# 530300865/Cooperative-ORB-SLAM

Measured on AMD Instinct MI355X. Metric: frames/sec ORB extract+match, 640x480 mono, 1000 feat/frame, higher is better.
Workload: dtype u8; 1 GPU; C2: synthetic 640x480 uint8, nfeatures 1000, scale 1.2, 8 levels, FAST 20/7; extract + BF SearchForTriangulation vs previous frame + per-step keyframe BoW + slot all-gather & cross-agent SearchForTriangulation and SearchByBoW(KF,KF); config=c2, stereo=False, graphs_per_gpu=3, graph_stagger=every8, scene=shared, exchange_stream=graph 0's, parallelism=agent-per-gpu x1

## Files before the change

cooperative-orb-slam_amd/csrc/launch.h:

```cpp
#pragma once
#include <hip/hip_runtime.h>
#include <stdint.h>

#include "../../include/orbslam_amd.h"
#include "orb_device.h"
#include "orb_frame.h"
#include "orb_match.h"
#include "orb_slot.h"

namespace orbamd {

hipError_t launch_resize(const uint8_t* src, long long src_fstride, int src_pitch, int sw, int sh, uint8_t* dst,
                         long long dst_fstride, int dst_pitch, int dw, int dh, const int* coef, int xmax,
                         int simd_end, int nframes, hipStream_t st);
hipError_t launch_pyramid_frames(const uint8_t* frames, long long fstride, int pitch0, uint8_t* pyr,
                                 const ExtractParams& ep, const LevelDesc* levels, const int* ptab, int max_rows,
                                 int max_groups, int nframes, hipStream_t st,
                                 const int2* bands = nullptr, int nbands = 0);
hipError_t launch_resize_tiled(const uint8_t* src, long long src_fstride, int src_pitch, int sw, int sh, uint8_t* dst,
                               long long dst_fstride, int dst_pitch, int dw, int dh, const int* coef, int xmax,
                               int simd_end, int nframes, hipStream_t st);
int resize_tile_fits(const int* xofs, const int* yofs, int sw, int sh, int dw, int dh);
hipError_t launch_fast_cells2(const uint8_t* frames, long long fstride, int pitch0, const uint8_t* pyr,
                              const ExtractParams& ep, const LevelDesc* levels, const CellDesc* cells,
                              uint32_t* cellkey, int* cellcnt, int RP, int RH, int max_pass, int cell_lo,
                              int cell_hi, int nframes, hipStream_t st);
hipError_t octree_setup(int lds_bytes);
hipError_t launch_sincos_selftest(const float* in, float* so, float* co, int n, hipStream_t st);
hipError_t launch_octree(const ExtractParams& ep, const LevelDesc* levels, const CellDesc* cells,
                         const uint32_t* cellkey, const int* cellcnt, uint32_t* lvkey, int* lvcnt,
                         uint8_t* gscratch, long long gscratch_frame_bytes, int NC, int KL, int lds_bytes,
                         int* err, int nframes, hipStream_t st, int level0 = 0, int nlevels = -1,
                         const HostCopy* copy = nullptr);
hipError_t launch_fast_blur(const uint8_t* frames, long long fstride, int pitch0, const uint8_t* pyr,
                            const ExtractParams& ep, const LevelDesc* levels, const CellDesc* cells, uint32_t* cellkey,
                            int* cellcnt, int RP, int RH, int max_pass, uint8_t* blur, const ExtractParams& eb,
                            int njobs, int nframes, hipStream_t st);
hipError_t launch_blur_strips(const uint8_t* frames, long long fstride, int pitch0, const uint8_t* pyr, uint8_t* blur,
                              const ExtractParams& ep, const LevelDesc* levels, int job0, int job1, const int* lvcnt,
                              int nframes, hipStream_t st, int rows = kBlurRows);
hipError_t launch_describe(const uint8_t* frames, long long fstride, int pitch0, const uint8_t* pyr,
                           const uint8_t* blur, const ExtractParams& ep, const LevelDesc* levels,
                           const uint32_t* lvkey, const int* lvcnt, orbx_kp* out_kps, uint8_t* out_desc,
                           int* out_counts, int kp_stride, const int* ptab, int nframes, hipStream_t st);
bool describe_blur_ok(const uint8_t* frames, long long fstride, int pitch0);
hipError_t launch_describe_blur(const uint8_t* frames, long long fstride, int pitch0, const uint8_t* pyr,
                                const ExtractParams& ep, const LevelDesc* levels, const uint32_t* lvkey,
                                const int* lvcnt, orbx_kp* out_kps, uint8_t* out_desc, int* out_counts, int kp_stride,
                                const int* ptab, int nframes, hipStream_t st);

hipError_t launch_tri_bf(int npairs, const int32_t* q1, const int32_t* q2, const orbx_kp* kps, const uint8_t* desc,
                         const int32_t* counts, int kp_stride, const MatchGeom& g, int32_t* match12,
                         int32_t* nmatches, hipStream_t st, const float* uright = nullptr, int only_stereo = 0);
hipError_t launch_tri_nodes_pairs(int npairs, int max_nodes, const int32_t* q1, const int32_t* q2, const orbx_kp* kps,
                                  const uint8_t* desc, int kp_stride, const uint32_t* fv_node, const int32_t* fv_off,
                                  const int32_t* fv_feat, const int32_t* nfv, const MatchGeom& g, int32_t* match12,
                                  int32_t* nmatches, hipStream_t st);
hipError_t launch_rot_filter_pairs(int npairs, const int32_t* q1, const int32_t* q2, const orbx_kp* kps,
                                   const int32_t* counts, int kp_stride, int32_t* match12, int32_t* nmatches,
                                   hipStream_t st, int swap = 0);
hipError_t launch_bow_pairs(int npairs, int max_nodes, const int32_t* qf, const int32_t* cf, const uint8_t* desc,
                            int kp_stride, const uint8_t* mp_flags, const uint32_t* fv_node, const int32_t* fv_off,
                            const int32_t* fv_feat, const int32_t* nfv, float nnratio, int mode, int32_t* out,
                            hipStream_t st);
hipError_t launch_count_pairs(int npairs, const int32_t* out, int kp_stride, int32_t* nmatches, hipStream_t st);
hipError_t launch_tri_nodes(const DevView& v1, const DevView& v2, const NodeTask* tasks, int ntasks,
                            const MatchGeom& g, int only_stereo, const CallTail& tail, hipStream_t st);
hipError_t launch_bow(const DevView& vq, const DevView& vc, const NodeTask* tasks, int ntasks, int max_nc,
                      float nnratio, int mode, const CallTail& tail, hipStream_t st);
hipError_t launch_bow_small(const BowSmall& a, hipStream_t st);
int proj_topk();
hipError_t launch_tri_small(const TriSmall& a, hipStream_t st);
hipError_t launch_rot_filter(int n, int32_t* m, const float* angA, const float* angB, int swap, int32_t* nout,
                             hipStream_t st);

hipError_t launch_undistort(const orbx_camera& cam, int nframes, const orbx_kp* kps, const int32_t* counts,
                            int kp_stride, orbx_kp* kps_un, float* kun, hipStream_t st);
hipError_t launch_undistort_deliver(const orbx_camera& cam, const orbx_kp* kps, const int32_t* count, int kp_stride,
                                    orbx_kp* raw_out, orbx_kp* un_out, int32_t* count_out, hipStream_t st);

hipError_t launch_unproject(float cx, float cy, float invfx, float invfy, int nframes, const orbx_kp* kps_un,
                            const float* depth, const int32_t* counts, int kp_stride, const float* Tcw, float* pos,
                            uint8_t* mp_flags, int valid_flags, hipStream_t st);
struct TrackArgs {
    const int32_t *cur, *last;
    int nframes;
// ... 75 lines not shown
```

cooperative-orb-slam_amd/csrc/match_kernels.hip:

```cpp
#include <hip/hip_runtime.h>
#include <stdint.h>
#include <limits.h>

#include "../../include/orbslam_amd.h"
#include "orb_match.h"
#include "orb_match_dev.h"
#include "orb_wave.h"

namespace orbamd {

__device__ __forceinline__ bool epi_ok_f(float a, float b, float c, float x2, float y2, float thf) {
    const float num = __fadd_rn(__fadd_rn(__fmul_rn(a, x2), __fmul_rn(b, y2)), c);
    const float den = __fadd_rn(__fmul_rn(a, a), __fmul_rn(b, b));
    if (den == 0.f) return false;
    const float dsqr = __fdiv_rn(__fmul_rn(num, num), den);
    return dsqr < thf;
}

__device__ __forceinline__ void epi_line(const MatchGeom& g, float x1, float y1, float* a, float* b, float* c) {
    epi_line(g.F, x1, y1, a, b, c);
}
__device__ __forceinline__ bool near_epipole(const MatchGeom& g, float x2, float y2, int oct2) {
    return near_epipole(g.ex, g.ey, x2, y2, g.th100[oct2]);
}

struct PairSrc {
    const orbx_kp* kps1; const uint8_t* desc1; int n1;
    const orbx_kp* kps2; const uint8_t* desc2; int n2;
    const float* ur1; const float* ur2;
};

typedef int v4i __attribute__((ext_vector_type(4)));

typedef int v8i __attribute__((ext_vector_type(8)));
typedef float v16f __attribute__((ext_vector_type(16)));
__device__ __forceinline__ uint32_t fp4_pm1_byte(uint32_t nb) {
    const uint32_t lo = nb & 15u, hi = (nb >> 4) & 15u;
    return ((hi * 0x10204080u) & 0x80808080u) | (((lo * 0x01020408u) & 0x08080808u) | 0x22222222u);
}
// ... 98 lines not shown
            auto key = [&](int p) {
                const float dp = __int_as_float(p & ~31);
                return ((uint32_t)(int)(256.f - dp) >> 1 << 16) + kb - (uint32_t)(p & 31);
            };
            int pmax = pk(0);
#pragma unroll
            for (int rg = 1; rg < 16; rg++) pmax = max(pmax, pk(rg));
            uint32_t km = key(pmax);
            while (km < best && (km >> 16) <= 50u) {
                const int jl = (int)(65535u - (km & 0xFFFFu)) - cb;
                const float4 c2 = s_rec[bf][jl];
                if ((!STEREO || st1 || c2.w == 0.0f) && epi_ok_f(la, lb, lc, c2.x, c2.y, c2.z)) {
                    best = km;
                    break;
                }
                const int cur = pmax;
                int nx = INT_MIN;
#pragma unroll
                for (int rg = 0; rg < 16; rg++) nx = pk(rg) < cur ? max(nx, pk(rg)) : nx;
                pmax = nx;
                km = nx == INT_MIN ? 0xFFFFFFFFu : key(nx);
            }
        }
        __syncthreads();
    }
    best = min(best, (uint32_t)__shfl_xor((int)best, 32, 64));
    if (qon && h == 0) {
        const int idx2 = qact && (best >> 16) <= 50u ? (int)(65535u - (best & 0xFFFFu)) : -1;
        out[qi] = idx2;
        if (idx2 >= 0) atomicAdd(nmatch, 1);
    }
}

#ifndef ORBX_MF_WPE
#define ORBX_MF_WPE 6
#endif
#define ORBX_MF_ATTR __attribute__((amdgpu_waves_per_eu(ORBX_MF_WPE)))
template <bool STEREO>
__global__ __launch_bounds__(kMfThreads) ORBX_MF_ATTR void k_tri_mfma(const int32_t* __restrict__ q1, const int32_t* __restrict__ q2,
                                                  const orbx_kp* __restrict__ kps, const uint8_t* __restrict__ desc,
                                                  const int32_t* __restrict__ counts, const float* __restrict__ uright,
                                                  int kp_stride, MatchGeom g, int only_stereo,
                                                  int32_t* __restrict__ match12, int32_t* __restrict__ nmatches) {
    const int p = blockIdx.y;
    const int f1 = q1[p], f2 = q2[p];
    PairSrc s;
    s.kps1 = kps + (long long)f1 * kp_stride; s.desc1 = desc + (long long)f1 * kp_stride * 32; s.n1 = counts[f1];
    s.kps2 = kps + (long long)f2 * kp_stride; s.desc2 = desc + (long long)f2 * kp_stride * 32; s.n2 = counts[f2];
    s.ur1 = STEREO ? uright + (long long)f1 * kp_stride : nullptr;
    s.ur2 = STEREO ? uright + (long long)f2 * kp_stride : nullptr;
    tri_mfma_body_fp4<STEREO>(s, g, match12 + (long long)p * kp_stride, nmatches + p, only_stereo);
}

__device__ __forceinline__ int rot_bin(const float* angA, const float* angB, int i, int j, int swap) {
    return swap ? rot_bin(angA[j], angB[i]) : rot_bin(angA[i], angB[j]);
}

__device__ __forceinline__ void call_emit(const CallTail& t, int i, int j) {
    const int bin = t.check_ori ? rot_bin(t.angA, t.angB, i, j, t.swap) : 0;
    if (t.check_ori) atomicAdd(t.state + 2 + bin, 1);
    const int k = atomicAdd(t.state + 1, 1);
    ((int4*)t.list)[k] = make_int4(i, j, bin, 0);
}

__device__ void call_tail(const CallTail& t) {
    __shared__ int s_last, s_cnt, s_nl;
    __shared__ int hist[30], keep[3];
    __syncthreads();
    __threadfence();
    if (threadIdx.x == 0) s_last = atomicAdd(t.state, 1) == (int)(gridDim.x - 1);
    __syncthreads();
    if (!s_last) return;
    __threadfence();
    if (threadIdx.x < 30) hist[threadIdx.x] = t.check_ori ? t.state[2 + threadIdx.x] : 0;
    if (threadIdx.x == 0) {
        s_cnt = 0;
        s_nl = t.state[1];
    }
    __syncthreads();
    if (threadIdx.x == 0) {
        if (t.check_ori) three_maxima(hist, keep);
        else keep[0] = keep[1] = keep[2] = -2;
    }
    __syncthreads();
// ... 390 lines not shown

__global__ __launch_bounds__(256) void k_rot_filter(int n, int32_t* __restrict__ m, const float* __restrict__ angA,
                                                    const float* __restrict__ angB, int swap, int32_t* __restrict__ nout) {
    __shared__ int hist[30];
    __shared__ int keep[3];
    const int local = rot_filter_rows(n, m, [&](int i, int j) { return rot_bin(angA, angB, i, j, swap); }, hist, keep);
    if (nout) atomicAdd(nout, local);
}

__global__ __launch_bounds__(256) void k_rot_filter_pairs(const int32_t* __restrict__ q1, const int32_t* __restrict__ q2,
                                                          const orbx_kp* __restrict__ kps, const int32_t* __restrict__ counts,
                                                          int kp_stride, int32_t* __restrict__ match12,
                                                          int32_t* __restrict__ nmatches, int swap) {
    __shared__ int hist[30];
    __shared__ int keep[3];
    const int p = blockIdx.x;
    const orbx_kp* k1 = kps + (long long)q1[p] * kp_stride;
    const orbx_kp* k2 = kps + (long long)q2[p] * kp_stride;
    if (threadIdx.x == 0) nmatches[p] = 0;
    const int local = rot_filter_rows(counts[q1[p]], match12 + (long long)p * kp_stride, [&](int i, int j) {
        return swap ? rot_bin(k2[j].angle, k1[i].angle) : rot_bin(k1[i].angle, k2[j].angle);
    }, hist, keep);
    atomicAdd(&nmatches[p], local);
}

}

#include "launch.h"

namespace orbamd {

hipError_t launch_tri_bf(int npairs, const int32_t* q1, const int32_t* q2, const orbx_kp* kps, const uint8_t* desc,
                         const int32_t* counts, int kp_stride, const MatchGeom& g, int32_t* match12,
                         int32_t* nmatches, hipStream_t st, const float* uright, int only_stereo) {
    if (npairs == 0) return hipSuccess;
    dim3 grid((kp_stride + 32 * kMfWaves - 1) / (32 * kMfWaves), npairs);
    if (uright)
        hipLaunchKernelGGL(k_tri_mfma<true>, grid, dim3(kMfThreads), 0, st, q1, q2, kps, desc, counts, uright, kp_stride,
                           g, only_stereo, match12, nmatches);
    else
        hipLaunchKernelGGL(k_tri_mfma<false>, grid, dim3(kMfThreads), 0, st, q1, q2, kps, desc, counts, uright,
                           kp_stride, g, 0, match12, nmatches);
    return hipGetLastError();
}

hipError_t launch_tri_nodes_pairs(int npairs, int max_nodes, const int32_t* q1, const int32_t* q2, const orbx_kp* kps,
                                  const uint8_t* desc, int kp_stride, const uint32_t* fv_node, const int32_t* fv_off,
                                  const int32_t* fv_feat, const int32_t* nfv, const MatchGeom& g, int32_t* match12,
                                  int32_t* nmatches, hipStream_t st) {
    if (npairs == 0 || max_nodes <= 0) return hipSuccess;
    hipLaunchKernelGGL(k_tri_nodes_pairs, dim3(max_nodes, npairs), dim3(64), 0, st, q1, q2, kps, desc, kp_stride,
                       fv_node, fv_off, fv_feat, nfv, g, match12, nmatches);
    return hipGetLastError();
}

hipError_t launch_rot_filter_pairs(int npairs, const int32_t* q1, const int32_t* q2, const orbx_kp* kps,
                                   const int32_t* counts, int kp_stride, int32_t* match12, int32_t* nmatches,
                                   hipStream_t st, int swap) {
    hipLaunchKernelGGL(k_rot_filter_pairs, dim3(npairs), dim3(256), 0, st, q1, q2, kps, counts, kp_stride, match12,
                       nmatches, swap);
    return hipGetLastError();
}

hipError_t launch_bow_pairs(int npairs, int max_nodes, const int32_t* qf, const int32_t* cf, const uint8_t* desc,
                            int kp_stride, const uint8_t* mp_flags, const uint32_t* fv_node, const int32_t* fv_off,
                            const int32_t* fv_feat, const int32_t* nfv, float nnratio, int mode, int32_t* out,
                            hipStream_t st) {
    if (npairs == 0 || max_nodes <= 0) return hipSuccess;
    hipLaunchKernelGGL(k_bow_pairs, dim3(max_nodes, npairs), dim3(64), (size_t)kp_stride, st, qf, cf, desc, kp_stride,
                       mp_flags, fv_node, fv_off, fv_feat, nfv, nnratio, mode, out);
    return hipGetLastError();
}

hipError_t launch_count_pairs(int npairs, const int32_t* out, int kp_stride, int32_t* nmatches, hipStream_t st) {
    if (npairs == 0) return hipSuccess;
// ... 42 lines not shown
```

cooperative-orb-slam_amd/csrc/matcher.cpp:

```cpp
#include "matcher_host.h"

using namespace orbamd;

namespace {

int wait_call(hipStream_t st, const int32_t* word) {
    return wait_until(st, [word] { return __atomic_load_n(word, __ATOMIC_ACQUIRE) >= 0; });
}

void make_geom(MatchGeom& g, const float F12[9], float ex, float ey, int nlevels, const float* scale,
               const float* sigma2) {
    for (int i = 0; i < 9; i++) g.F[i] = F12[i];
    g.ex = ex;
    g.ey = ey;
    for (int o = 0; o < 16; o++) {
        g.th100[o] = o < nlevels ? 100 * scale[o] : 0.f;
        g.th384[o] = o < nlevels ? 3.84 * (double)sigma2[o] : 0.0;
        float t = (float)g.th384[o];
        if ((double)t < g.th384[o]) t = std::nextafter(t, INFINITY);
        g.th384f[o] = t;
    }
}

void common_nodes(const orbm_kf_view* a, const orbm_kf_view* b, std::vector<std::pair<int, int>>& out) {
// ... 80 lines not shown
        if (p.octave != none) memcpy(hbase + p.octave, v->octave, 4 * n);
        if (p.uright != none) memcpy(hbase + p.uright, v->uright, 4 * n);
        if (v->has_mp) memcpy(hbase + p.has_mp, v->has_mp, n);
        if (v->mp_bad) memcpy(hbase + p.mp_bad, v->mp_bad, n);
    }
    if (p.nfeat) memcpy(hbase + p.feat, v->node_feat, 4 * (size_t)p.nfeat);
    return d;
}

}

extern "C" {

int orbm_create(int device, orbm_ctx** out) {
    if (!out) return ORBX_EARG;
    *out = nullptr;
    if (device < 0 || device >= orbx_device_count()) return ORBX_EDEVICE;
    HIPR(hipSetDevice(device));
    orbm_ctx* c = new orbm_ctx();
    c->device = device;
    if (c->err.ensure(256) || hipMemset(c->err.p, 0, 256) != hipSuccess) {
        orbm_destroy(c);
        return ORBX_EDEVICE;
    }
    *out = c;
    return 0;
}

void orbm_destroy(orbm_ctx* c) {
    if (!c) return;
    (void)hipSetDevice(c->device);
    if (c->stream) (void)hipStreamSynchronize(c->stream);
    c->scratch.release();
    c->err.release();
    if (c->pinned) (void)hipHostFree(c->pinned);
    if (c->stream) (void)hipStreamDestroy(c->stream);
    delete c;
}

int orbm_descriptor_distance(const uint8_t* a, const uint8_t* b) {
    if (!a || !b) return ORBX_EARG;
    int d = 0;
    for (int i = 0; i < 8; i++) {
        uint32_t x, y;
        memcpy(&x, a + 4 * i, 4);
        memcpy(&y, b + 4 * i, 4);
        d += __builtin_popcount(x ^ y);
    }
    return d;
}

void orbm_epipole(const float R2w[9], const float t2w[3], const float Cw[3], float fx, float fy, float cx, float cy,
                  float* ex, float* ey) {
    float C2[3];
    for (int i = 0; i < 3; i++) {
        const float* a = R2w + 3 * i;
        const float t0 = a[0] * Cw[0] + a[1] * Cw[1] + a[2] * Cw[2];
        C2[i] = (float)((double)t0 * 1.0 + (double)t2w[i] * 1.0);
    }
    const float invz = 1.0f / C2[2];
    *ex = fx * C2[0] * invz + cx;
    *ey = fy * C2[1] * invz + cy;
}

}

static int node_feats(const orbm_kf_view* v) { return v->n_nodes ? v->node_off[v->n_nodes] : 0; }

struct SmallSide {
    const uint4* d = nullptr;
// ... 281 lines not shown
    HIPR(launch_bow(dq, dc, (const NodeTask*)(base + o_tasks), (int)tasks.size(), max_nc, nnratio, mode, tail,
                    ctx->s()));
    if (const int rc = wait_call(ctx->s(), res)) return rc;
    memcpy(out, res + 1, 4 * (size_t)nout);
    if (nmatches) *nmatches = res[0];
    return 0;
}

int orbm_search_by_bow_kf_f(orbm_ctx* ctx, const orbm_kf_view* kf, const orbm_kf_view* f, float nnratio,
                            int check_ori, int32_t* match_f, int* nmatches) {
    if (!ctx || !view_ok(kf) || !view_ok(f) || !match_f) return ORBX_EARG;
    return bow_common(ctx, kf, f, nnratio, check_ori, 0, match_f, f->n, nmatches);
}

int orbm_search_by_bow_kf_kf(orbm_ctx* ctx, const orbm_kf_view* kf1, const orbm_kf_view* kf2, float nnratio,
                             int check_ori, int32_t* match12, int* nmatches) {
    if (!ctx || !view_ok(kf1) || !view_ok(kf2) || !match12) return ORBX_EARG;
    return bow_common(ctx, kf1, kf2, nnratio, check_ori, 1, match12, kf1->n, nmatches);
}

int orbm_triangulation_bf_batch_device(orbm_ctx* ctx, int npairs, const int32_t* d_q1, const int32_t* d_q2,
                                       const orbx_kp* d_kps, const uint8_t* d_desc, const int32_t* d_counts,
                                       int kp_stride, const float F12[9], float ex, float ey, int nlevels,
                                       const float* scale_factors, const float* level_sigma2, int check_ori,
                                       int32_t* d_match12, int32_t* d_nmatches, void* stream) {
    if (!ctx || npairs < 0 || !F12 || nlevels < 1 || nlevels > 16 || !scale_factors || !level_sigma2 ||
        kp_stride < 1 || kp_stride > 64 * 1024)
        return ORBX_EARG;
    if (npairs == 0) return 0;
    HIPR(hipSetDevice(ctx->device));
    MatchGeom g;
    make_geom(g, F12, ex, ey, nlevels, scale_factors, level_sigma2);
    hipStream_t st = (hipStream_t)stream;
    HIPR(hipMemsetAsync(d_nmatches, 0, sizeof(int32_t) * npairs, st));
    HIPR(launch_tri_bf(npairs, d_q1, d_q2, d_kps, d_desc, d_counts, kp_stride, g, d_match12, d_nmatches, st));
    if (check_ori)
        HIPR(launch_rot_filter_pairs(npairs, d_q1, d_q2, d_kps, d_counts, kp_stride, d_match12, d_nmatches, st));
    return 0;
}

int orbm_triangulation_bf_stereo_batch_device(orbm_ctx* ctx, int npairs, const int32_t* d_q1, const int32_t* d_q2,
                                              const orbx_kp* d_kps, const uint8_t* d_desc, const int32_t* d_counts,
                                              const float* d_uright, int kp_stride, const float F12[9], float ex,
                                              float ey, int nlevels, const float* scale_factors,
                                              const float* level_sigma2, int only_stereo, int check_ori,
                                              int32_t* d_match12, int32_t* d_nmatches, void* stream) {
    if (!ctx || npairs < 0 || !F12 || nlevels < 1 || nlevels > 16 || !scale_factors || !level_sigma2 ||
        kp_stride < 1 || kp_stride > 64 * 1024 || (npairs > 0 && !d_uright))
        return ORBX_EARG;
    if (npairs == 0) return 0;
    HIPR(hipSetDevice(ctx->device));
    MatchGeom g;
    make_geom(g, F12, ex, ey, nlevels, scale_factors, level_sigma2);
    hipStream_t st = (hipStream_t)stream;
    HIPR(hipMemsetAsync(d_nmatches, 0, sizeof(int32_t) * npairs, st));
    HIPR(launch_tri_bf(npairs, d_q1, d_q2, d_kps, d_desc, d_counts, kp_stride, g, d_match12, d_nmatches, st, d_uright,
                       only_stereo ? 1 : 0));
    if (check_ori)
        HIPR(launch_rot_filter_pairs(npairs, d_q1, d_q2, d_kps, d_counts, kp_stride, d_match12, d_nmatches, st));
    return 0;
}

int orbm_triangulation_nodes_batch_device(orbm_ctx* ctx, int npairs, const int32_t* d_q1, const int32_t* d_q2,
                                          const orbx_kp* d_kps, const uint8_t* d_desc, const int32_t* d_counts,
                                          int kp_stride, const uint32_t* d_fv_node, const int32_t* d_fv_off,
                                          const int32_t* d_fv_feat, const int32_t* d_nfv, int max_nodes,
                                          const float F12[9], float ex, float ey, int nlevels,
                                          const float* scale_factors, const float* level_sigma2, int check_ori,
                                          int32_t* d_match12, int32_t* d_nmatches, void* stream) {
    if (!ctx || npairs < 0 || !F12 || nlevels < 1 || nlevels > 16 || !scale_factors || !level_sigma2 ||
        kp_stride < 1 || max_nodes < 0 || max_nodes > kp_stride)
        return ORBX_EARG;
    if (npairs == 0) return 0;
    HIPR(hipSetDevice(ctx->device));
    MatchGeom g;
    make_geom(g, F12, ex, ey, nlevels, scale_factors, level_sigma2);
    hipStream_t st = (hipStream_t)stream;
    HIPR(hipMemsetAsync(d_match12, 0xFF, sizeof(int32_t) * (size_t)npairs * kp_stride, st));
    HIPR(hipMemsetAsync(d_nmatches, 0, sizeof(int32_t) * npairs, st));
    HIPR(launch_tri_nodes_pairs(npairs, max_nodes, d_q1, d_q2, d_kps, d_desc, kp_stride, d_fv_node, d_fv_off,
                                d_fv_feat, d_nfv, g, d_match12, d_nmatches, st));
    if (check_ori)
        HIPR(launch_rot_filter_pairs(npairs, d_q1, d_q2, d_kps, d_counts, kp_stride, d_match12, d_nmatches, st));
    return 0;
}

int orbm_search_by_bow_batch_device(orbm_ctx* ctx, int npairs, int mode, const int32_t* d_qf, const int32_t* d_cf,
                                    const orbx_kp* d_kps, const uint8_t* d_desc, const int32_t* d_counts,
                                    int kp_stride, const uint8_t* d_mp_flags, const uint32_t* d_fv_node,
                                    const int32_t* d_fv_off, const int32_t* d_fv_feat, const int32_t* d_nfv,
// ... 185 lines not shown
```

cooperative-orb-slam_amd/csrc/matcher_host.h:

```cpp
#pragma once
#include <memory>
#include <vector>

#include "host_util.h"
#include "kf_cache.h"
#include "launch.h"

struct orbm_ctx {
    int device = 0;
    hipStream_t stream = nullptr;
    int ready() {
        HIPR(hipSetDevice(device));
        if (!stream && hipStreamCreateWithFlags(&stream, hipStreamNonBlocking) != hipSuccess) {
            stream = nullptr;
            return ORBX_EDEVICE;
        }
        return 0;
    }
    hipStream_t s() const { return stream; }
    orbamd::DevBuf scratch;
    orbamd::DevBuf err;
    std::vector<uint8_t> host;
    void* pinned = nullptr;
    void* pinned_dev = nullptr;
    size_t pinned_bytes = 0;
    uint8_t* ensure_pinned(size_t need) {
        if (need <= pinned_bytes) return (uint8_t*)pinned;
        if (stream) (void)hipStreamSynchronize(stream);
        if (pinned) (void)hipHostFree(pinned);
        pinned = nullptr;
        pinned_dev = nullptr;
        pinned_bytes = 0;
        if (hipHostMalloc(&pinned, need, hipHostMallocCoherent) != hipSuccess) return nullptr;
        if (hipHostGetDevicePointer(&pinned_dev, pinned, 0) != hipSuccess) {
            (void)hipHostFree(pinned);
            pinned = nullptr;
            return nullptr;
        }
        pinned_bytes = need;
        return (uint8_t*)pinned;
    }
    int32_t* pinned_on_device(size_t off) const { return (int32_t*)((uint8_t*)pinned_dev + off); }
    uint32_t seq = 0;
    uint32_t next_seq() {
        seq = seq >= orbamd::kSmallSeqMask ? 1u : seq + 1u;
        return seq;
    }
    int32_t* call_state() { return err.as<int32_t>() + 16; }
};

namespace orbamd {

struct KfEntry {
    DevBuf buf;
    int n = 0, nfeat = 0, n_nodes = 0;
    bool has_ur = false, has_grid = false;
    size_t o_desc = 0, o_x = 0, o_y = 0, o_ang = 0, o_oct = 0, o_ur = 0, o_feat = 0, o_gs = 0, o_gi = 0;
    size_t o_dnode = 0, o_rnode = 0;
    float min_x = 0, min_y = 0, gw_inv = 0, gh_inv = 0;
    const uint8_t* at(size_t o) const { return buf.as<uint8_t>() + o; }
    size_t bytes() const { return buf.bytes; }
};

}

struct orbm_kf_cache {
    int device = 0;
    hipStream_t stream = nullptr;
    orbamd::KfLru<orbamd::KfEntry> lru;
    explicit orbm_kf_cache(size_t capacity) : lru(capacity) {}
};

namespace orbamd {
std::shared_ptr<KfEntry> cache_get(orbm_kf_cache* c, int kind, uint64_t key, const orbm_kf_view* kv,
                                   const orbm_frame_view* fv, hipStream_t st);
}
```

cooperative-orb-slam_amd/csrc/orbslam_amd_testing.h:

```cpp
#ifndef ORBSLAM_AMD_TESTING_H
#define ORBSLAM_AMD_TESTING_H
#include "../../include/orbslam_amd.h"

#ifdef __cplusplus
extern "C" {
#endif

int orbx_debug_skip_stages(orbx_handle* h, int mask);

int orbx_debug_serial(orbx_handle* h, int on);

int orbx_debug_alias_frames(orbx_handle* h, int on);

int orbx_debug_raise_error(orbx_handle* h, int flag, void* stream);

int orbx_debug_hip_failure(void);

int orbx_describe_blur_fused(const void* frames, size_t frame_stride, size_t pitch);

int orbx_selftest_sincosf(const float* d_in, float* d_sin, float* d_cos, int n, void* stream);

int orbx_selftest_logf(const float* d_in, float* d_out, int n, void* stream);

#ifdef __cplusplus
}
#endif
#endif
```

cooperative-orb-slam_amd/orbamd/_lib.py:

```python
import ctypes as C
import os

PKG_DIR = os.path.dirname(os.path.dirname(os.path.abspath(__file__)))
_VARIANT = os.environ.get("ORBAMD_LIB_VARIANT", "")
LIB_PATH = os.path.join(PKG_DIR, "lib", "liborbamd%s.so" % ("_" + _VARIANT if _VARIANT else ""))

ORBX_OK = 0
ORBX_EARG = -1
ORBX_EDEVICE = -2
ORBX_ECAPACITY = -3


class OrbxParams(C.Structure):
    _fields_ = [("nfeatures", C.c_int32), ("scale_factor", C.c_float), ("nlevels", C.c_int32),
                ("ini_th_fast", C.c_int32), ("min_th_fast", C.c_int32)]


class OrbxKp(C.Structure):
    _fields_ = [("x", C.c_float), ("y", C.c_float), ("size", C.c_float), ("angle", C.c_float),
                ("response", C.c_float), ("octave", C.c_int32)]


class OrbxCamera(C.Structure):
    _fields_ = [(k, C.c_float) for k in ("fx", "fy", "cx", "cy", "k1", "k2", "p1", "p2", "k3")]
# ... 64 lines not shown
_I = C.c_int
_F = C.c_float
_SZ = C.c_size_t
SIGNATURES = {
    "orbx_create": (_I, [C.POINTER(OrbxParams), _I, _I, _I, _I, C.POINTER(_P)]),
    "orbx_destroy": (None, [_P]),
    "orbx_max_keypoints": (_I, [_P, _I, _I]),
    "orbx_extract": (_I, [_P, _P, _I, _I, _SZ, _P, _P, _I, C.POINTER(_I)]),
    "orbx_extract_batch_device": (_I, [_P, _I, _P, _SZ, _I, _I, _SZ, _P, _P, _P, _I, _P]),
    "orbx_pyramid_level": (_I, [_P, _I, _I, _P, _SZ, C.POINTER(_I), C.POINTER(_I)]),
    "orbx_set_host_pyramid": (_I, [_P, _I]),
    "orbx_host_pyramid_level": (_I, [_P, _I, C.POINTER(_P), C.POINTER(_SZ), C.POINTER(_I), C.POINTER(_I)]),
    "orbx_host_pyramid_bytes": (_I, [_P, _I, _I, C.POINTER(_SZ)]),
    "orbx_host_register": (_I, [_P, _SZ]),
    "orbx_host_unregister": (_I, [_P]),
    "orbx_set_host_pyramid_target": (_I, [_P, _P, _SZ]),
    "orbx_get_levels": (_I, [_P]),
    "orbx_get_scale_factor": (_F, [_P]),
    "orbx_get_scale_tables": (_I, [_P, _P, _P, _P, _P]),
    "orbx_get_feature_split": (_I, [_P, _P, _P]),
    "orbx_compute_scale_tables": (_I, [C.POINTER(OrbxParams), _P, _P, _P, _P]),
    "orbx_set_pyramid_event": (_I, [_P, _P]),
    "orbx_set_stage_event": (_I, [_P, _I, _P]),
    "orbx_debug_skip_stages": (_I, [_P, _I]),
    "orbx_debug_hip_failure": (_I, []),
    "orbx_comm_unique_id": (_I, [_P]),
    "orbx_comm_create": (_I, [_P, _I, _I, _I, _P]),
    "orbx_comm_allgather": (_I, [_P, _P, _P, _SZ, _P]),
    "orbx_comm_destroy": (None, [_P]),
    "orbx_describe_blur_fused": (_I, [_P, _SZ, _SZ]),
    "orbx_debug_serial": (_I, [_P, _I]),
    "orbx_debug_alias_frames": (_I, [_P, _I]),
    "orbx_debug_raise_error": (_I, [_P, _I, _P]),
    "orbm_create": (_I, [_I, C.POINTER(_P)]),
    "orbm_destroy": (None, [_P]),
    "orbm_descriptor_distance": (_I, [_P, _P]),
    "orbm_search_for_triangulation": (_I, [_P, C.POINTER(OrbmKfView), C.POINTER(OrbmKfView), _P, _F, _F, _I, _I,
                                           _P, C.POINTER(_I)]),
    "orbm_search_by_bow_kf_f": (_I, [_P, C.POINTER(OrbmKfView), C.POINTER(OrbmKfView), _F, _I, _P, C.POINTER(_I)]),
    "orbm_search_by_bow_kf_kf": (_I, [_P, C.POINTER(OrbmKfView), C.POINTER(OrbmKfView), _F, _I, _P, C.POINTER(_I)]),
    "orbm_triangulation_bf_batch_device": (_I, [_P, _I, _P, _P, _P, _P, _P, _I, _P, _F, _F, _I, _P, _P, _I, _P, _P,
                                                _P]),
    "orbm_triangulation_bf_stereo_batch_device": (_I, [_P, _I, _P, _P, _P, _P, _P, _P, _I, _P, _F, _F, _I, _P, _P, _I,
                                                       _I, _P, _P, _P]),
    "orbm_search_for_triangulation_slots_device": (_I, [_P, C.POINTER(OrbxKfSource), _I, _I, _P, _SZ,
                                                        C.POINTER(OrbmSlotGeom), _I, _I, _P, _P, _P]),
    "orbm_search_by_bow_slots_device": (_I, [_P, C.POINTER(OrbxKfSource), _I, _I, _P, _SZ, _F, _I, _I, _P, _P, _P]),
    "orbm_check_error": (_I, [_P, _P]),
    "orbm_triangulation_nodes_batch_device": (_I, [_P, _I, _P, _P, _P, _P, _P, _I, _P, _P, _P, _P, _I, _P, _F, _F,
                                                   _I, _P, _P, _I, _P, _P, _P]),
    "orbm_search_by_bow_batch_device": (_I, [_P, _I, _I, _P, _P, _P, _P, _P, _I, _P, _P, _P, _P, _P, _I, _F, _I, _P,
                                             _P, _P]),
    "orbm_epipole": (None, [_P, _P, _P, _F, _F, _F, _F, C.POINTER(_F), C.POINTER(_F)]),
    "orbx_slot_bytes": (_SZ, [_I]),
    "orbx_slot_layout": (_I, [_I, C.POINTER(OrbxSlotHeader)]),
    "orbx_pack_keyframe_device": (_I, [C.POINTER(OrbxKfSource), C.POINTER(OrbxKfMeta), _I, _P, _P, _P]),
    "orbx_pack_keyframe_host": (_I, [C.POINTER(OrbxKfSource), C.POINTER(OrbxKfMeta), _I, _P, _SZ]),
    "orbx_slot_parse": (_I, [_P, _SZ, C.POINTER(OrbxSlotView)]),
    "orbx_synth_frame": (_I, [_I, _I, _I, _I, _P]),
    "orbx_synth_frames": (_I, [_I, _I, _I, _I, _I, _P]),
    "orbx_synth_frames_shifted": (_I, [_I, _I, _I, _I, _I, _I, _P]),
    "orbx_synth_scene_frames": (_I, [_I, _I, _I, _I, _I, _I, _I, _P]),
    "orbx_compute_stereo_matches": (_I, [_P, _P, _P, _P, _I, _P, _P, _I, _F, _F, _P, _P, C.POINTER(_I)]),
    "orbx_stereo_matches_batch_device": (_I, [_P, _P, _I, _P, _P, _P, _P, _P, _P, _P, _P, _I, _F, _F, _P, _P, _P,
                                              _P]),
    "orbx_check_error": (_I, [_P, _P]),
# ... 102 lines not shown
```

Baseline: 405,500 frames/s.

## Cull epipolar-impossible candidate tiles in brute-force triangulation matcher

Adds a pre-pass kernel that orders query and candidate keypoints along the epipolar-line direction with a bitonic sort in LDS. It groups candidates into 32-point tiles with bounding boxes and thresholds, and gathers their descriptors into a permuted scratch layout. The MFMA matcher then uses a conservative bbox-to-line distance test per wave to skip chunks and tiles that no query in the block can match epipolarly. This avoids MFMA Hamming work and selection on impossible candidates, at the cost of an extra sort and gather kernel, scratch memory, and more synchronisation.

Measured after the change: 426,100 frames/s (median of 6 runs). 5.1% higher.

```diff
diff --git a/cooperative-orb-slam_amd/csrc/launch.h b/cooperative-orb-slam_amd/csrc/launch.h
--- a/cooperative-orb-slam_amd/csrc/launch.h
+++ b/cooperative-orb-slam_amd/csrc/launch.h
@@ -7,6 +7,7 @@
 #include "orb_frame.h"
 #include "orb_match.h"
 #include "orb_slot.h"
+#include "orb_tri_cull.h"
 
 namespace orbamd {
 
@@ -51,7 +52,8 @@
 
 hipError_t launch_tri_bf(int npairs, const int32_t* q1, const int32_t* q2, const orbx_kp* kps, const uint8_t* desc,
                          const int32_t* counts, int kp_stride, const MatchGeom& g, int32_t* match12,
-                         int32_t* nmatches, hipStream_t st, const float* uright = nullptr, int only_stereo = 0);
+                         int32_t* nmatches, hipStream_t st, const float* uright = nullptr, int only_stereo = 0,
+                         const TriPlan* plan = nullptr);
 hipError_t launch_tri_nodes_pairs(int npairs, int max_nodes, const int32_t* q1, const int32_t* q2, const orbx_kp* kps,
                                   const uint8_t* desc, int kp_stride, const uint32_t* fv_node, const int32_t* fv_off,
                                   const int32_t* fv_feat, const int32_t* nfv, const MatchGeom& g, int32_t* match12,
diff --git a/cooperative-orb-slam_amd/csrc/match_kernels.hip b/cooperative-orb-slam_amd/csrc/match_kernels.hip
--- a/cooperative-orb-slam_amd/csrc/match_kernels.hip
+++ b/cooperative-orb-slam_amd/csrc/match_kernels.hip
@@ -5,6 +5,7 @@
 #include "../../include/orbslam_amd.h"
 #include "orb_match.h"
 #include "orb_match_dev.h"
+#include "orb_tri_cull.h"
 #include "orb_wave.h"
 
 namespace orbamd {
@@ -169,16 +170,276 @@
     }
 }
 
+constexpr int kMfMaxChunks = kTriOrdCap / kMfChunk;
+static_assert(kMfMaxChunks <= 64, "the needed-chunk list is compacted by one wave's ballot");
+static_assert(kMfChunk == 2 * kTriTile, "a chunk is two tiles, one per lane half of the cull ballot");
+
+template <bool STEREO>
+__device__ __forceinline__ void tri_mfma_body_cull(const PairSrc& s, const MatchGeom& g, const uint16_t* __restrict__ permQ,
+                                                   const uint8_t* __restrict__ sdesc, const float4* __restrict__ srec,
+                                                   const TriTile* __restrict__ tiles, unsigned long long* stats,
+                                                   int32_t* __restrict__ out, int32_t* __restrict__ nmatch,
+                                                   int only_stereo) {
+    static_assert(kMfWaves == 4 || kMfWaves == 8, "fp4 expansion roles: 4 waves (2 dwords per thread) or 8 (1)");
+    constexpr int kDw = 512 / kMfThreads;
+    __shared__ v4i s_frag[kMfBufs][2][4][64];
+    __shared__ float4 s_rec[kMfBufs][kMfChunk];
+    __shared__ float4 s_box[2 * kMfMaxChunks];
+    __shared__ float s_thf[2 * kMfMaxChunks];
+    __shared__ uint8_t s_need[kMfWaves][kMfMaxChunks];
+    __shared__ uint8_t s_list[kMfMaxChunks];
+    __shared__ int s_nlist;
+    const int tid = threadIdx.x, wave = tid >> 6, lane = tid & 63;
+    const int qblk = blockIdx.x * (32 * kMfWaves);
+    if (qblk >= s.n1) return;
+    if (s.n2 <= 0) {
+        if (tid < 32 * kMfWaves && qblk + tid < s.n1) out[permQ[qblk + tid]] = -1;
+        return;
+    }
+    const int h = lane >> 5;
+    const int qpos = qblk + wave * 32 + (lane & 31);
+    const bool qon = qpos < s.n1;
+    const int qi = qon ? (int)permQ[qpos] : 0;
+    const bool st1 = STEREO && qon && s.ur1[qi] >= 0.f;
+    const bool qact = qon && (!STEREO || !only_stereo || st1);
+    v4i bq[4];
+    float la = 0.f, lb = 0.f, lc = 0.f;
+    {
+        const uint4* qd = (const uint4*)(s.desc1 + (long long)qi * 32);
+        const uint4 d0 = qd[0], d1 = qd[1];
+        const uint32_t dw[8] = {d0.x, d0.y, d0.z, d0.w, d1.x, d1.y, d1.z, d1.w};
+#pragma unroll
+        for (int st = 0; st < 4; st++) bq[st] = fp4_pm1_dword(h ? dw[2 * st + 1] : dw[2 * st]);
+        const orbx_kp k1 = s.kps1[qi];
+        epi_line(g, k1.x, k1.y, &la, &lb, &lc);
+    }
+    const int ntiles = (s.n2 + kTriTile - 1) / kTriTile, nchunks = (s.n2 + kMfChunk - 1) / kMfChunk;
+    if (tid < 2 * nchunks) {
+        const int tt = min(tid, ntiles - 1);
+        s_box[tid] = *(const float4*)&tiles[tt].xmin;
+        s_thf[tid] = tid < ntiles ? tiles[tt].thf : -1.f;
+    }
+    __syncthreads();
+    for (int c = 0; c < nchunks; c++) {
+        const float4 bx = s_box[2 * c + h];
+        const TriTile tl = {bx.x, bx.y, bx.z, bx.w, s_thf[2 * c + h], 0.f, 0.f, 0.f};
+        const bool alive = qact && !tri_tile_dead(la, lb, lc, tl);
+        const unsigned long long b = __ballot(alive);
+        if (lane == 0) s_need[wave][c] = (uint8_t)(((uint32_t)b != 0u ? 1 : 0) | ((uint32_t)(b >> 32) != 0u ? 2 : 0));
+    }
+    __syncthreads();
+    if (wave == 0) {
+        int any = 0;
+        if (lane < nchunks)
+            for (int w = 0; w < kMfWaves; w++) any |= s_need[w][lane];
+        const unsigned long long m = __ballot(any != 0);
+        if (any) s_list[__popcll(m & ((1ull << lane) - 1ull))] = (uint8_t)lane;
+        if (lane == 0) s_nlist = __popcll(m);
+    }
+    __syncthreads();
+    const int nl = s_nlist;
+    uint32_t best = 0xFFFFFFFFu;
+    const int ec = (tid >> 6) * (64 / kMfWaves) + (tid & 7) + (kDw == 1 ? 0 : 8 * ((tid >> 5) & 1));
+    const int ed = kDw == 1 ? (tid >> 3) & 7 : 2 * ((tid >> 3) & 3);
+    struct DwT { uint32_t w[kDw]; };
+    DwT pd;
+    float4 pr = make_float4(0.f, 0.f, -1.f, 0.f);
+    auto load_chunk = [&](int cb) {
+        const int c = min(cb + ec, s.n2 - 1);
+        pd = *(const DwT*)(sdesc + (long long)c * 32 + 4 * ed);
+        if (tid < kMfChunk) pr = srec[min(cb + tid, s.n2 - 1)];
+    };
+    auto stage = [&](int cbw, int bw) {
+        const bool on = cbw + ec < s.n2;
+        const int tile = ec >> 5, r = ec & 31;
+#pragma unroll
+        for (int k = 0; k < kDw; k++)
+            s_frag[bw][tile][(ed + k) >> 1][32 * ((ed + k) & 1) + r] = fp4_pm1_dword(on ? pd.w[k] : 0u);
+        if (tid < kMfChunk) s_rec[bw][tid] = cbw + tid < s.n2 ? pr : make_float4(0.f, 0.f, -1.0f, 0.f);
+    };
+    int nexec = 0;
+    if (nl > 0) {
+        load_chunk(kMfChunk * s_list[0]);
+        stage(kMfChunk * s_list[0], 0);
+        __syncthreads();
+        if (nl > 1) load_chunk(kMfChunk * s_list[1]);
+    }
+    for (int k = 0, bf = 0; k < nl; k++, bf ^= 1) {
+        if (k + 1 < nl) {
+            stage(kMfChunk * s_list[k + 1], bf ^ 1);
+            if (k + 2 < nl) load_chunk(kMfChunk * s_list[k + 2]);
+        }
+        auto select = [&](const v16f& acc, int tile) {
+            auto pk = [&](int rg) { return __float_as_int(acc[rg]) | ((rg & 3) + 8 * (rg >> 2)); };
+            auto dist = [&](int pv) { return (uint32_t)(int)(256.f - __int_as_float(pv & ~31)) >> 1; };
+            int pmax = pk(0);
+#pragma unroll
+            for (int rg = 1; rg < 16; rg++) pmax = max(pmax, pk(rg));
+            uint32_t D = dist(pmax);
+            while (D <= (best >> 16) && D <= 50u) {
+                const float4 c2 = s_rec[bf][32 * tile + 4 * h + (pmax & 31)];
+                const uint32_t bits = __float_as_uint(c2.w);
+                const uint32_t km = (D << 16) | (65535u - (bits & 0xFFFFu));
+                if (km >= best) break;
+                if ((!STEREO || st1 || (bits >> 16) == 0u) && epi_ok_f(la, lb, lc, c2.x, c2.y, c2.z)) {
+                    best = km;
+                    break;
+                }
+                const int cur = pmax;
+                int nx = INT_MIN;
+#pragma unroll
+                for (int rg = 0; rg < 16; rg++) nx = pk(rg) < cur ? max(nx, pk(rg)) : nx;
+                pmax = nx;
+                D = nx == INT_MIN ? 0xFFFFu : dist(nx);
+            }
+        };
+        const int nb = __builtin_amdgcn_readfirstlane((int)s_need[wave][s_list[k]]);
+        nexec += __popc(nb);
+#pragma unroll
+        for (int tile = 0; tile < 2; tile++) {
+            if (!(nb >> tile & 1)) continue;
+            v16f acc = (v16f)0.f;
+#pragma unroll
+            for (int st = 0; st < 4; st++)
+                acc = __builtin_amdgcn_mfma_scale_f32_32x32x64_f8f6f4(fp4_operand(s_frag[bf][tile][st][lane]), fp4_operand(bq[st]),
+                                                                      acc, 4, 4, 0, 127, 0, 127);
+            select(acc, tile);
+        }
+        __syncthreads();
+    }
+    best = min(best, (uint32_t)__shfl_xor((int)best, 32, 64));
+    if (qon && h == 0) {
+        const int idx2 = qact && (best >> 16) <= 50u ? (int)(65535u - (best & 0xFFFFu)) : -1;
+        out[qi] = idx2;
+        if (idx2 >= 0) atomicAdd(nmatch, 1);
+    }
+    if (stats && __ballot(qon) != 0ull && lane == 0) {
+        atomicAdd(stats, (unsigned long long)nexec);
+        atomicAdd(stats + 1, (unsigned long long)ntiles);
+    }
+}
+
+constexpr int kOrdThreads = 512;
+
+__device__ __forceinline__ void lds_sort2_u32(uint32_t* sa, uint32_t* sb, int npad) {
+    bool wide_prev = true;
+    for (int k = 2; k <= npad; k <<= 1)
+        for (int j = k >> 1; j > 0; j >>= 1) {
+            const bool wide = j >= 128;
+            if (wide || wide_prev) __syncthreads();
+            else __builtin_amdgcn_fence(__ATOMIC_ACQ_REL, "workgroup");
+            wide_prev = wide;
+            for (int i = threadIdx.x; i < (npad >> 1); i += kOrdThreads) {
+                const int lo = ((i & ~(j - 1)) << 1) | (i & (j - 1)), hi = lo | j;
+                const bool up = (lo & k) == 0;
+                const uint32_t a = sa[lo], b = sa[hi], c = sb[lo], d = sb[hi];
+                if ((a > b) == up) {
+                    sa[lo] = b;
+                    sa[hi] = a;
+                }
+                if ((c > d) == up) {
+                    sb[lo] = d;
+                    sb[hi] = c;
+                }
+            }
+        }
+    __syncthreads();
+}
+
+template <bool STEREO>
+__global__ __launch_bounds__(kOrdThreads) void k_tri_order(const int32_t* __restrict__ q1, const int32_t* __restrict__ q2,
+                                                           const orbx_kp* __restrict__ kps, const uint8_t* __restrict__ desc,
+                                                           const int32_t* __restrict__ counts,
+                                                           const float* __restrict__ uright, int kp_stride, MatchGeom g,
+                                                           int only_stereo, TriPlan pl) {
+    __shared__ uint32_t s_kq[kTriOrdCap], s_key[kTriOrdCap];
+    __shared__ uint16_t s_perm[kTriOrdCap];
+    constexpr uint32_t kIdxMask = kTriOrdCap - 1;
+    const int p = blockIdx.x, tid = threadIdx.x;
+    const int f1 = q1[p], f2 = q2[p];
+    const int cap = min(kp_stride, min(pl.S, kTriOrdCap));
+    const int n1 = min(max(counts[f1], 0), cap), n2 = min(max(counts[f2], 0), cap);
+    const orbx_kp* k1 = kps + (long long)f1 * kp_stride;
+    const orbx_kp* k2 = kps + (long long)f2 * kp_stride;
+    const uint8_t* d2 = desc + (long long)f2 * kp_stride * 32;
+    const TriOrd o = tri_ord_make(g.F);
+    const long long row = (long long)p * pl.S;
+
+    int npad = 1;
+    while (npad < max(n1, n2)) npad <<= 1;
+    for (int i = tid; i < npad; i += kOrdThreads) {
+        uint32_t kq = 0xFFFFFFFFu, kc = 0xFFFFFFFFu;
+        if (i < n1) {
+            const orbx_kp kp = k1[i];
+            float a, b, c;
+            epi_line(g, kp.x, kp.y, &a, &b, &c);
+            kq = tri_query_key(o, a, b, c) << kTriOrdIdxBits | (uint32_t)i;
+        }
+        if (i < n2) {
+            const orbx_kp kp = k2[i];
+            kc = tri_cand_key(o, kp.x, kp.y) << kTriOrdIdxBits | (uint32_t)i;
+        }
+        s_kq[i] = kq;
+        s_key[i] = kc;
+    }
+    lds_sort2_u32(s_kq, s_key, npad);
+    for (int i = tid; i < n1; i += kOrdThreads) pl.permQ[row + i] = (uint16_t)(s_kq[i] & kIdxMask);
+    for (int i = tid; i < n2; i += kOrdThreads) {
+        const int tb = i & ~(kTriTile - 1), cnt = min(kTriTile, n2 - tb);
+        const uint32_t my = s_key[i] & kIdxMask;
+        int r = 0;
+        for (int k = 0; k < cnt; k++) r += (s_key[tb + k] & kIdxMask) < my;
+        s_perm[tb + r] = (uint16_t)my;
+    }
+    __syncthreads();
+    for (int base = 0; base < n2; base += kOrdThreads) {
+        const int i = base + tid;
+        const bool on = i < n2;
+        float x = 0.f, y = 0.f, thf = -1.f;
+        if (on) {
+            const int j = s_perm[i];
+            const orbx_kp kp = k2[j];
+            x = kp.x;
+            y = kp.y;
+            uint32_t near = 0u;
+            if (STEREO) {
+                const bool st2 = uright[(long long)f2 * kp_stride + j] >= 0.f;
+                near = !st2 && near_epipole(g, x, y, kp.octave) ? 1u : 0u;
+                thf = !only_stereo || st2 ? g.th384f[kp.octave] : -1.f;
+            } else {
+                thf = near_epipole(g, x, y, kp.octave) ? -1.f : g.th384f[kp.octave];
+            }
+            const uint4* sd = (const uint4*)(d2 + (long long)j * 32);
+            uint4* dd = (uint4*)(pl.sdesc + (row + i) * 32);
+            dd[0] = sd[0];
+            dd[1] = sd[1];
+            ((float4*)pl.srec)[row + i] = make_float4(x, y, thf, __uint_as_float((uint32_t)j | near << 16));
+        }
+        const bool live = on && thf >= 0.f;
+        TriTile t = {live ? x : INFINITY, live ? x : -INFINITY, live ? y : INFINITY, live ? y : -INFINITY,
+                     live ? thf : -1.f, 0.f, 0.f, 0.f};
+#pragma unroll
+        for (int w = kTriTile / 2; w > 0; w >>= 1) {
+            t.xmin = fminf(t.xmin, __shfl_xor(t.xmin, w, kTriTile));
+            t.xmax = fmaxf(t.xmax, __shfl_xor(t.xmax, w, kTriTile));
+            t.ymin = fminf(t.ymin, __shfl_xor(t.ymin, w, kTriTile));
+            t.ymax = fmaxf(t.ymax, __shfl_xor(t.ymax, w, kTriTile));
+            t.thf = fmaxf(t.thf, __shfl_xor(t.thf, w, kTriTile));
+        }
+        if (on && (tid & (kTriTile - 1)) == 0) pl.tiles[row / kTriTile + i / kTriTile] = t;
+    }
+}
+
 #ifndef ORBX_MF_WPE
 #define ORBX_MF_WPE 6
 #endif
 #define ORBX_MF_ATTR __attribute__((amdgpu_waves_per_eu(ORBX_MF_WPE)))
-template <bool STEREO>
+template <bool STEREO, bool CULL>
 __global__ __launch_bounds__(kMfThreads) ORBX_MF_ATTR void k_tri_mfma(const int32_t* __restrict__ q1, const int32_t* __restrict__ q2,
                                                   const orbx_kp* __restrict__ kps, const uint8_t* __restrict__ desc,
                                                   const int32_t* __restrict__ counts, const float* __restrict__ uright,
                                                   int kp_stride, MatchGeom g, int only_stereo,
-                                                  int32_t* __restrict__ match12, int32_t* __restrict__ nmatches) {
+                                                  int32_t* __restrict__ match12, int32_t* __restrict__ nmatches, TriPlan pl) {
     const int p = blockIdx.y;
     const int f1 = q1[p], f2 = q2[p];
     PairSrc s;
@@ -186,7 +447,17 @@
     s.kps2 = kps + (long long)f2 * kp_stride; s.desc2 = desc + (long long)f2 * kp_stride * 32; s.n2 = counts[f2];
     s.ur1 = STEREO ? uright + (long long)f1 * kp_stride : nullptr;
     s.ur2 = STEREO ? uright + (long long)f2 * kp_stride : nullptr;
-    tri_mfma_body_fp4<STEREO>(s, g, match12 + (long long)p * kp_stride, nmatches + p, only_stereo);
+    if constexpr (CULL) {
+        const int cap = min(kp_stride, min(pl.S, kTriOrdCap));
+        s.n1 = min(s.n1, cap);
+        s.n2 = min(s.n2, cap);
+        const long long row = (long long)p * pl.S;
+        tri_mfma_body_cull<STEREO>(s, g, pl.permQ + row, pl.sdesc + row * 32, (const float4*)pl.srec + row,
+                                   pl.tiles + row / kTriTile, pl.stats, match12 + (long long)p * kp_stride,
+                                   nmatches + p, only_stereo);
+    } else {
+        tri_mfma_body_fp4<STEREO>(s, g, match12 + (long long)p * kp_stride, nmatches + p, only_stereo);
+    }
 }
 
 __device__ __forceinline__ int rot_bin(const float* angA, const float* angB, int i, int j, int swap) {
@@ -643,15 +914,29 @@
 
 hipError_t launch_tri_bf(int npairs, const int32_t* q1, const int32_t* q2, const orbx_kp* kps, const uint8_t* desc,
                          const int32_t* counts, int kp_stride, const MatchGeom& g, int32_t* match12,
-                         int32_t* nmatches, hipStream_t st, const float* uright, int only_stereo) {
+                         int32_t* nmatches, hipStream_t st, const float* uright, int only_stereo, const TriPlan* plan) {
     if (npairs == 0) return hipSuccess;
     dim3 grid((kp_stride + 32 * kMfWaves - 1) / (32 * kMfWaves), npairs);
-    if (uright)
-        hipLaunchKernelGGL(k_tri_mfma<true>, grid, dim3(kMfThreads), 0, st, q1, q2, kps, desc, counts, uright, kp_stride,
-                           g, only_stereo, match12, nmatches);
-    else
-        hipLaunchKernelGGL(k_tri_mfma<false>, grid, dim3(kMfThreads), 0, st, q1, q2, kps, desc, counts, uright,
-                           kp_stride, g, 0, match12, nmatches);
+    if (plan && (kp_stride > kTriOrdCap || plan->S < kp_stride || plan->S % kMfChunk)) return hipErrorInvalidValue;
+    const TriPlan pl = plan ? *plan : TriPlan{};
+    if (!uright) only_stereo = 0;
+    if (plan) {
+        if (uright)
+            hipLaunchKernelGGL(k_tri_order<true>, dim3(npairs), dim3(kOrdThreads), 0, st, q1, q2, kps, desc, counts, uright,
+                               kp_stride, g, only_stereo, pl);
+        else
+            hipLaunchKernelGGL(k_tri_order<false>, dim3(npairs), dim3(kOrdThreads), 0, st, q1, q2, kps, desc, counts,
+                               uright, kp_stride, g, only_stereo, pl);
+        if (hipError_t e = hipGetLastError()) return e;
+    }
+#define ORBX_TRI_MFMA(ST, CU)                                                                                        \
+    hipLaunchKernelGGL((k_tri_mfma<ST, CU>), grid, dim3(kMfThreads), 0, st, q1, q2, kps, desc, counts, uright, kp_stride, \
+                       g, only_stereo, match12, nmatches, pl)
+    if (uright && plan) ORBX_TRI_MFMA(true, true);
+    else if (uright) ORBX_TRI_MFMA(true, false);
+    else if (plan) ORBX_TRI_MFMA(false, true);
+    else ORBX_TRI_MFMA(false, false);
+#undef ORBX_TRI_MFMA
     return hipGetLastError();
 }
 
diff --git a/cooperative-orb-slam_amd/csrc/matcher.cpp b/cooperative-orb-slam_amd/csrc/matcher.cpp
--- a/cooperative-orb-slam_amd/csrc/matcher.cpp
+++ b/cooperative-orb-slam_amd/csrc/matcher.cpp
@@ -136,10 +136,35 @@
     (void)hipSetDevice(c->device);
     if (c->stream) (void)hipStreamSynchronize(c->stream);
     c->scratch.release();
+    c->tri_scratch.release();
+    c->tri_stats.release();
     c->err.release();
     if (c->pinned) (void)hipHostFree(c->pinned);
     if (c->stream) (void)hipStreamDestroy(c->stream);
     delete c;
+}
+
+int orbm_debug_tri_cull(orbm_ctx* ctx, int mode) {
+    if (!ctx || mode < 0 || mode > 2) return ORBX_EARG;
+    HIPR(hipSetDevice(ctx->device));
+    if (mode == 2) {
+        if (ctx->tri_stats.ensure(2 * sizeof(unsigned long long))) return ORBX_EDEVICE;
+        HIPR(hipDeviceSynchronize());
+        HIPR(hipMemset(ctx->tri_stats.p, 0, 2 * sizeof(unsigned long long)));
+    }
+    ctx->tri_cull = mode;
+    return 0;
+}
+
+int orbm_debug_tri_cull_counts(orbm_ctx* ctx, unsigned long long out[2]) {
+    if (!ctx || !out) return ORBX_EARG;
+    out[0] = out[1] = 0;
+    if (!ctx->tri_stats.p) return 0;
+    HIPR(hipSetDevice(ctx->device));
+    HIPR(hipDeviceSynchronize());
+    HIPR(hipMemcpy(out, ctx->tri_stats.p, 2 * sizeof(unsigned long long), hipMemcpyDeviceToHost));
+    HIPR(hipMemset(ctx->tri_stats.p, 0, 2 * sizeof(unsigned long long)));
+    return 0;
 }
 
 int orbm_descriptor_distance(const uint8_t* a, const uint8_t* b) {
@@ -487,8 +512,13 @@
     MatchGeom g;
     make_geom(g, F12, ex, ey, nlevels, scale_factors, level_sigma2);
     hipStream_t st = (hipStream_t)stream;
+    TriPlan pl;
+    const bool cull = ctx->tri_culled(kp_stride);
+    if (cull)
+        if (const int rc = ctx->tri_plan(npairs, kp_stride, pl)) return rc;
     HIPR(hipMemsetAsync(d_nmatches, 0, sizeof(int32_t) * npairs, st));
-    HIPR(launch_tri_bf(npairs, d_q1, d_q2, d_kps, d_desc, d_counts, kp_stride, g, d_match12, d_nmatches, st));
+    HIPR(launch_tri_bf(npairs, d_q1, d_q2, d_kps, d_desc, d_counts, kp_stride, g, d_match12, d_nmatches, st, nullptr, 0,
+                       cull ? &pl : nullptr));
     if (check_ori)
         HIPR(launch_rot_filter_pairs(npairs, d_q1, d_q2, d_kps, d_counts, kp_stride, d_match12, d_nmatches, st));
     return 0;
@@ -508,9 +538,13 @@
     MatchGeom g;
     make_geom(g, F12, ex, ey, nlevels, scale_factors, level_sigma2);
     hipStream_t st = (hipStream_t)stream;
+    TriPlan pl;
+    const bool cull = ctx->tri_culled(kp_stride);
+    if (cull)
+        if (const int rc = ctx->tri_plan(npairs, kp_stride, pl)) return rc;
     HIPR(hipMemsetAsync(d_nmatches, 0, sizeof(int32_t) * npairs, st));
     HIPR(launch_tri_bf(npairs, d_q1, d_q2, d_kps, d_desc, d_counts, kp_stride, g, d_match12, d_nmatches, st, d_uright,
-                       only_stereo ? 1 : 0));
+                       only_stereo ? 1 : 0, cull ? &pl : nullptr));
     if (check_ori)
         HIPR(launch_rot_filter_pairs(npairs, d_q1, d_q2, d_kps, d_counts, kp_stride, d_match12, d_nmatches, st));
     return 0;
diff --git a/cooperative-orb-slam_amd/csrc/matcher_host.h b/cooperative-orb-slam_amd/csrc/matcher_host.h
--- a/cooperative-orb-slam_amd/csrc/matcher_host.h
+++ b/cooperative-orb-slam_amd/csrc/matcher_host.h
@@ -47,6 +47,24 @@
         return seq;
     }
     int32_t* call_state() { return err.as<int32_t>() + 16; }
+    orbamd::DevBuf tri_scratch, tri_stats;
+    int tri_cull = 1;
+    bool tri_culled(int kp_stride) const { return tri_cull && kp_stride <= orbamd::kTriOrdCap; }
+    int tri_plan(int npairs, int kp_stride, orbamd::TriPlan& pl) {
+        orbamd::Carve cv;
+        const size_t S = (size_t)orbamd::align_up(kp_stride, 64), rows = (size_t)npairs * S;
+        const size_t o_perm = cv.take(rows * sizeof(uint16_t)), o_desc = cv.take(rows * 32);
+        const size_t o_rec = cv.take(rows * 16), o_tile = cv.take(rows / orbamd::kTriTile * sizeof(orbamd::TriTile));
+        if (tri_scratch.ensure(cv.off)) return ORBX_EDEVICE;
+        uint8_t* b = tri_scratch.as<uint8_t>();
+        pl.permQ = (uint16_t*)(b + o_perm);
+        pl.sdesc = b + o_desc;
+        pl.srec = (float*)(b + o_rec);
+        pl.tiles = (orbamd::TriTile*)(b + o_tile);
+        pl.stats = tri_cull == 2 ? tri_stats.as<unsigned long long>() : nullptr;
+        pl.S = (int)S;
+        return 0;
+    }
 };
 
 namespace orbamd {
diff --git a/cooperative-orb-slam_amd/csrc/orb_tri_cull.h b/cooperative-orb-slam_amd/csrc/orb_tri_cull.h
--- /dev/null
+++ b/cooperative-orb-slam_amd/csrc/orb_tri_cull.h
@@ -0,0 +1,92 @@
+#pragma once
+#include <math.h>
+#include <stdint.h>
+
+#if defined(__HIPCC__)
+#define ORB_HD __host__ __device__ inline
+#else
+#define ORB_HD inline
+#endif
+
+namespace orbamd {
+
+constexpr int kTriOrdIdxBits = 12;
+constexpr int kTriOrdCap = 1 << kTriOrdIdxBits;
+constexpr int kTriTile = 32;
+
+struct TriTile {
+    float xmin, xmax, ymin, ymax, thf, pad0, pad1, pad2;
+};
+
+struct TriPlan {
+    uint16_t* permQ;
+    uint8_t* sdesc;
+    float* srec;
+    TriTile* tiles;
+    unsigned long long* stats;
+    int S;
+};
+
+struct TriOrd {
+    float nx, ny, ux, uy, kappa, c0x, c0y;
+};
+
+ORB_HD TriOrd tri_ord_make(const float* F) {
+    float s = 0.f, G[9];
+    for (int i = 0; i < 9; i++) s = fmaxf(s, fabsf(F[i]));
+    for (int i = 0; i < 9; i++) G[i] = F[i] / s;
+    float best = -1.f, ex = 0.f, ey = 0.f, ew = 0.f;
+    for (int i = 0; i < 3; i++) {
+        const float* r0 = G + 3 * i;
+        const float* r1 = G + 3 * ((i + 1) % 3);
+        const float cx = r0[1] * r1[2] - r0[2] * r1[1], cy = r0[2] * r1[0] - r0[0] * r1[2];
+        const float cw = r0[0] * r1[1] - r0[1] * r1[0];
+        const float nn = cx * cx + cy * cy + cw * cw;
+        if (nn > best) { best = nn; ex = cx; ey = cy; ew = cw; }
+    }
+    TriOrd o;
+    o.c0x = 0.f;
+    o.c0y = 0.f;
+    if (ex * ex + ey * ey < 4096.f * ew * ew) o.c0x = 1024.f;
+    const float dx = ex - ew * o.c0x, dy = ey - ew * o.c0y;
+    const float L = sqrtf(dx * dx + dy * dy);
+    o.nx = dx / L;
+    o.ny = dy / L;
+    o.ux = -o.ny;
+    o.uy = o.nx;
+    o.kappa = ew / L;
+    return o;
+}
+
+ORB_HD uint32_t tri_ord_key(float t) {
+    float g = t / (fabsf(t) + 512.f) + 1.f;
+    if (!(g >= 0.f)) g = 0.f;
+    if (g > 2.f) g = 2.f;
+    return (uint32_t)(g * 524287.5f);
+}
+ORB_HD uint32_t tri_cand_key(const TriOrd& o, float x, float y) {
+    const float dx = x - o.c0x, dy = y - o.c0y;
+    return tri_ord_key((o.ux * dx + o.uy * dy) / (1.f - o.kappa * (o.nx * dx + o.ny * dy)));
+}
+ORB_HD uint32_t tri_query_key(const TriOrd& o, float a, float b, float c) {
+    const float rz = -(o.nx * o.c0x + o.ny * o.c0y);
+    const float px = b * rz - c * o.ny, py = c * o.nx - a * rz, pw = a * o.ny - b * o.nx;
+    return tri_ord_key((o.ux * px + o.uy * py) / pw - (o.ux * o.c0x + o.uy * o.c0y));
+}
+
+ORB_HD bool tri_tile_dead(float a, float b, float c, const TriTile& t) {
+    const float den = a * a + b * b;
+    if (den == 0.f || t.thf < 0.f) return true;
+    if (!(den >= 1e-30f && den <= 1e30f)) return false;
+    const float v0 = a * t.xmin + b * t.ymin + c, v1 = a * t.xmax + b * t.ymin + c;
+    const float v2 = a * t.xmin + b * t.ymax + c, v3 = a * t.xmax + b * t.ymax + c;
+    float m = 0.f;
+    if (v0 > 0.f && v1 > 0.f && v2 > 0.f && v3 > 0.f) m = fminf(fminf(v0, v1), fminf(v2, v3));
+    else if (v0 < 0.f && v1 < 0.f && v2 < 0.f && v3 < 0.f) m = -fmaxf(fmaxf(v0, v1), fmaxf(v2, v3));
+    const float X = fmaxf(fabsf(t.xmin), fabsf(t.xmax)), Y = fmaxf(fabsf(t.ymin), fabsf(t.ymax));
+    const float E = fabsf(a) * X + fabsf(b) * Y + fabsf(c);
+    const float mm = m - 6.103515625e-5f * E;
+    return mm > 0.f && mm * mm > t.thf * den * 1.0001220703125f;
+}
+
+}
diff --git a/cooperative-orb-slam_amd/csrc/orbslam_amd_testing.h b/cooperative-orb-slam_amd/csrc/orbslam_amd_testing.h
--- a/cooperative-orb-slam_amd/csrc/orbslam_amd_testing.h
+++ b/cooperative-orb-slam_amd/csrc/orbslam_amd_testing.h
@@ -22,6 +22,10 @@
 
 int orbx_selftest_logf(const float* d_in, float* d_out, int n, void* stream);
 
+int orbm_debug_tri_cull(orbm_ctx* ctx, int mode);
+
+int orbm_debug_tri_cull_counts(orbm_ctx* ctx, unsigned long long out[2]);
+
 #ifdef __cplusplus
 }
 #endif
diff --git a/cooperative-orb-slam_amd/orbamd/_lib.py b/cooperative-orb-slam_amd/orbamd/_lib.py
--- a/cooperative-orb-slam_amd/orbamd/_lib.py
+++ b/cooperative-orb-slam_amd/orbamd/_lib.py
@@ -120,6 +120,8 @@
     "orbx_debug_serial": (_I, [_P, _I]),
     "orbx_debug_alias_frames": (_I, [_P, _I]),
     "orbx_debug_raise_error": (_I, [_P, _I, _P]),
+    "orbm_debug_tri_cull": (_I, [_P, _I]),
+    "orbm_debug_tri_cull_counts": (_I, [_P, _P]),
     "orbm_create": (_I, [_I, C.POINTER(_P)]),
     "orbm_destroy": (None, [_P]),
     "orbm_descriptor_distance": (_I, [_P, _P]),
```
